# kanster/moped

Measured on AMD Instinct MI355X. Metric: detections/sec (frames/s) 640x480 ~3k SIFT vs N models, higher is better.
Workload: dtype f32

## Files before the change

include/moped_hip.h:

```cpp
#ifndef MOPED_HIP_H
#define MOPED_HIP_H

#include <stddef.h>
#include <stdint.h>

#ifdef __cplusplus
extern "C" {
#endif

#define MH_DESC_DIM 128
#define MH_MAX_BATCH 32
#define MH_MAX_IMAGES 8
#define MH_MAX_MODELS 8192
#define MH_OK 0
#define MH_ERR_ARG (-1)
#define MH_ERR_HIP (-2)
#define MH_ERR_CAPACITY (-3)
#define MH_ERR_NODEVICE (-4)

typedef struct mh_ctx mh_ctx;


int mh_create(int device, mh_ctx** out);
void mh_destroy(mh_ctx* ctx);
// ... 23 lines not shown
int mh_match_stats(mh_ctx* ctx, int Q, uint32_t stats[4], int reset);
int mh_match_set_mode(mh_ctx* ctx, int mode);
int mh_pose_set_split(mh_ctx* ctx, int on);
int mh_match_launches(mh_ctx* ctx, uint32_t out[3]);
float mh_screen_margin(float qq, float dmax);
int mh_screen_values(mh_ctx* ctx, const float* q_host, int Q, int n_rows, float* out_host, float* dmax, float* spread,
                     int shape );
uint16_t mh_screen_record_value(float top, float thr);
void mh_screen_record_bounds(uint16_t value_bits, uint32_t row0, float tau, float spread, int N, float dmax, float* lo,
                             float* hi);
float mh_screen_pack_value(float v, uint32_t id, int bits);
float mh_screen_pack_pert(float qq, float dmax, int bits);
void mh_screen_sample_bounds(uint16_t value_bits, float tau, float pert, float dmax, float* lo, float* hi);
void mh_screen_launch_plan(int Q, int q_expected, int N, int32_t out[8]);
int mh_match_incomplete(mh_ctx* ctx, uint32_t* count, int reset);

int mh_match_local_dev(mh_ctx* ctx, const float* qn_dev, const float* qnorm_dev, int Q,
                       int32_t* idx1_dev, float* d1_dev, float* d2_dev);
int mh_match_merge_dev(mh_ctx* ctx, const int32_t* idx1_s_dev, const float* d1_s_dev,
                       const float* d2_s_dev, int n_shards, int Q,
                       int32_t* idx1_dev, float* d1_dev, float* d2_dev);
int mh_normalize_dev(mh_ctx* ctx, float* q_dev, float* qnorm_dev, int Q);


int mh_meanshift(mh_ctx* ctx, const float* pts_host, int n, int dim, float radius,
                 float merge, int min_pts, int max_iter, int32_t* label,
                 int32_t* order, int32_t* n_clusters);
int mh_meanshift_batch(mh_ctx* ctx, const float* pts_host, const int32_t* off, int n_problems,
                       int dim, float radius, float merge, int min_pts, int max_iter,
                       int32_t* label, int32_t* order, int32_t* n_clusters);
// ... 295 lines not shown
```

moped_amd/capi.py:

```python
from __future__ import annotations

import ctypes as C
import os

import numpy as np

_HERE = os.path.dirname(os.path.abspath(__file__))
LIB_PATH = os.environ.get("MH_LIB_PATH") or os.path.join(_HERE, "libmoped_hip.so")

MH_OK = 0


class MhError(RuntimeError):
    pass


class mh_corr(C.Structure):
    _fields_ = [("u", C.c_float), ("v", C.c_float), ("x", C.c_float), ("y", C.c_float), ("z", C.c_float)]


class mh_cam(C.Structure):
    _fields_ = [("K", C.c_float * 4), ("cam", C.c_float * 7)]


# ... 78 lines not shown
    "mh_db_upload_raw", "mh_db_share", "mh_match_stats", "mh_match_set_mode", "mh_match_launches", "mh_pose_set_split", "mh_frame_fetch_match_points", "mh_screen_margin", "mh_frame_counters", "mh_match_timing", "mh_frame_set_images", "mh_filter_images",
    "mh_pose_ransac_images",
    "mh_comm_unique_id", "mh_comm_create", "mh_comm_create_all", "mh_comm_create_host", "mh_comm_destroy", "mh_comm_info",
    "mh_frame_enqueue_sharded", "mh_frame_enqueue_sharded_batch", "mh_frame_enqueue_sharded_all",
    "mh_frame_previous_objects", "mh_frame_gather_objects", "mh_frame_enqueue_batch", "mh_frame_set_depth_image_batch",
    "mh_pose_kernel_info", "mh_db_upload_blocks", "mh_frame_fetch_matches_slot", "mh_frame_fetch_match_reps_slot",
    "mh_screen_values", "mh_screen_record_value", "mh_screen_record_bounds", "mh_reserve_batch", "mh_frame_run_host",
    "mh_frame_block_stride", "mh_frame_fetch_batch_async", "mh_frame_fetch_previous_async", "mh_frame_fetch_wait",
    "mh_frame_fetch_query", "mh_host_alloc", "mh_host_free", "mh_frame_run_host_begin", "mh_frame_wait_descriptors",
    "mh_step_match", "mh_step_match_fetch", "mh_step_cluster", "mh_step_pose", "mh_step_filter",
    "mh_set_linkage_scratch_limit",
    "mh_undistort_map", "mh_undistort", "mh_undistort_dev", "mh_frame_set_undistort",
    "mh_sift_extract_batch_dev", "mh_sift_debug_plan", "mh_sift_debug_level", "mh_sift_debug_candidates",
    "mh_sift_debug_keys", "mh_sift_debug_blur",
    "mh_screen_pack_value", "mh_screen_pack_pert", "mh_screen_sample_bounds", "mh_screen_launch_plan", "mh_match_incomplete",
]
COMM_ID_BYTES = 128
EX2_OBJECTS = 62
ALLGATHER_FN = C.CFUNCTYPE(C.c_int, C.c_void_p, C.c_void_p, C.c_void_p, C.c_size_t)

_lib = None


def load():
    global _lib
    if _lib is not None:
        return _lib
    try:
        import torch
    except Exception:
# ... 135 lines not shown
    L.mh_screen_values.argtypes = [vp, vp, i32, i32, vp, C.POINTER(f32), C.POINTER(f32), i32]
    L.mh_screen_record_value.argtypes = [f32, f32]
    L.mh_screen_record_value.restype = C.c_uint16
    L.mh_screen_record_bounds.argtypes = [C.c_uint16, C.c_uint32, f32, f32, i32, f32, C.POINTER(f32), C.POINTER(f32)]
    L.mh_screen_record_bounds.restype = None
    if hasattr(L, "mh_screen_pack_value"):
        L.mh_screen_pack_value.argtypes = [f32, C.c_uint32, i32]
        L.mh_screen_pack_value.restype = f32
        L.mh_screen_pack_pert.argtypes = [f32, f32, i32]
        L.mh_screen_pack_pert.restype = f32
        L.mh_screen_sample_bounds.argtypes = [C.c_uint16, f32, f32, f32, C.POINTER(f32), C.POINTER(f32)]
        L.mh_screen_sample_bounds.restype = None
        L.mh_screen_launch_plan.argtypes = [i32, i32, i32, vp]
        L.mh_screen_launch_plan.restype = None
        L.mh_match_incomplete.argtypes = [vp, C.POINTER(C.c_uint32), i32]
    L.mh_db_upload_blocks.argtypes = [vp, vp, vp, vp, i32, i32, vp, vp, i32, i32]
    L.mh_frame_block_stride.argtypes = [i32]
    L.mh_frame_block_stride.restype = C.c_size_t
    L.mh_frame_fetch_batch_async.argtypes = [vp, i32, i32, vp, C.c_uint32]
    L.mh_frame_fetch_previous_async.argtypes = [vp, i32, vp, C.c_uint32]
    L.mh_frame_fetch_wait.argtypes = [vp, C.POINTER(C.c_int32)]
    L.mh_host_alloc.argtypes = [vp, C.c_size_t, C.POINTER(vp)]
    L.mh_host_free.argtypes = [vp, vp]
    L.mh_frame_wait_descriptors.argtypes = [vp]
    if hasattr(L, "mh_step_match"):
        L.mh_set_linkage_scratch_limit.argtypes = [vp, C.c_size_t]
        L.mh_step_match.argtypes = [vp, vp, vp, i32, C.POINTER(mh_cam), f32, i32]
        L.mh_step_match_fetch.argtypes = [vp, vp, vp, vp, i32, C.POINTER(C.c_int32)]
        L.mh_step_cluster.argtypes = [vp, f32, f32, i32, i32, vp, vp, vp, i32, i32, C.POINTER(C.c_int32)]
        L.mh_step_pose.argtypes = [vp, i32, C.POINTER(mh_pose_params), C.c_uint64, vp, i32, C.POINTER(C.c_int32)]
# ... 263 lines not shown
                "waves_per_simd": int(o[3]) * waves / 4.0}

    def match_timing(self) -> dict:
        t = np.zeros(5, np.float32)
        self._ck(self.L.mh_match_timing(self.h, _ptr(t)), "mh_match_timing")
        return dict(zip(("prepare_ms", "pass_a_ms", "thresholds_ms", "pass_b_ms", "pass_c_ms"), (float(v) for v in t)))

    def screen_values(self, qn, n_rows, shape=0):
        qn = np.ascontiguousarray(qn, np.float32)
        out = np.zeros((qn.shape[0], n_rows), np.float32)
        dmax, spread = C.c_float(0), C.c_float(0)
        self._ck(self.L.mh_screen_values(self.h, _ptr(qn), qn.shape[0], n_rows, _ptr(out), C.byref(dmax), C.byref(spread),
                                         int(shape)), "mh_screen_values")
        return out, dmax.value, spread.value

    def match_set_mode(self, mode: int):
        self._ck(self.L.mh_match_set_mode(self.h, int(mode)), "mh_match_set_mode")

    def pose_set_split(self, on: bool):
        self._ck(self.L.mh_pose_set_split(self.h, int(bool(on))), "mh_pose_set_split")

    def match_kernel_launches(self) -> dict:
        o = np.zeros(3, np.uint32)
        self._ck(self.L.mh_match_launches(self.h, _ptr(o)), "mh_match_launches")
        return {"valu": int(o[0]), "mfma": int(o[1]), "screen": int(o[2])}

    def match_stats(self, Q=0, reset=False) -> dict:
        st = np.zeros(4, np.uint32)
        self._ck(self.L.mh_match_stats(self.h, int(Q), _ptr(st), int(reset)), "mh_match_stats")
        return {"candidates": int(st[0]), "brute_force_queries": int(st[1]), "queries": int(st[2]),
                "two_stage": bool(st[3])}

    def match_incomplete(self, reset=False) -> int:
        n = C.c_uint32(0)
        self._ck(self.L.mh_match_incomplete(self.h, C.byref(n), int(reset)), "mh_match_incomplete")
        return int(n.value)

    def normalize(self, desc):
        d = np.ascontiguousarray(desc, np.float32).copy()
        self._ck(self.L.mh_normalize(self.h, _ptr(d), d.shape[0]), "mh_normalize")
        return d

    def match(self, q, ratio=0.8):
        q = np.ascontiguousarray(q, np.float32)
        Q = q.shape[0]
        acc = np.full(Q, -1, np.int32)
# ... 701 lines not shown
```

moped_amd/csrc/api.hip:

```cpp
#include <algorithm>
#include <cmath>
#include <cstring>
#include <new>
#include <vector>

#include "context.h"
#include "steps.h"

using namespace mh;

namespace mh {

int use_stream(mh_ctx* ctx) {
  if (ctx->stream) return MH_OK;
  if (!ctx->own_stream) MH_HIP(ctx, hipStreamCreateWithFlags(&ctx->own_stream, hipStreamNonBlocking));
  ctx->stream = ctx->own_stream;
  return MH_OK;
}

int ensure_scratch(mh_ctx* ctx, size_t bytes) {
  if (bytes <= ctx->scratch_cap) return MH_OK;
  if (ctx->scratch) MH_HIP(ctx, hipFree(ctx->scratch));
  ctx->scratch = nullptr;
  ctx->scratch_cap = 0;
// ... 626 lines not shown
  hipMemcpyAsync(qd, q_host, (size_t)Q * DIM * 4, hipMemcpyHostToDevice, ctx->stream);
  launch_row_norms(qd, qn, Q, ctx->stream);
  launch_screen_prepare(qd, qn, Q, q_pad, qh, qbad, ctx->stream);
  launch_screen_values(qh, Q, ctx->sdb, n_rows, out, ctx->stream, shape);
  if (hipMemcpyAsync(out_host, out, (size_t)Q * n_rows * 4, hipMemcpyDeviceToHost, ctx->stream) != hipSuccess ||
      hipStreamSynchronize(ctx->stream) != hipSuccess || hipGetLastError() != hipSuccess) {
    ctx->err = "mh_screen_values: device error";
    rc = MH_ERR_HIP;
  }
  done();
  if (dmax) *dmax = ctx->sdb.dmax;
  if (spread) *spread = ctx->sdb.spread;
  return rc;
}

int mh_match_set_mode(mh_ctx* ctx, int mode) {
  if (!ctx || mode < -1 || mode > 3) return MH_ERR_ARG;
  ctx->match_mode = mode;
  return MH_OK;
}

int mh_pose_set_split(mh_ctx* ctx, int on) {
  if (!ctx) return MH_ERR_ARG;
  ctx->pose_split = on ? 1 : 0;
  return MH_OK;
}

int mh_match_launches(mh_ctx* ctx, uint32_t out[3]) {
  if (!ctx || !out) return MH_ERR_ARG;
  for (int k = 0; k < 3; ++k) out[k] = ctx->match_launches[k];
// ... 7 lines not shown
  stats[0] = stats[1] = stats[2] = stats[3] = 0;
  if (Q > 0) {
    int rc = ensure_match_scratch(ctx, Q);
    if (rc) return rc;
    stats[3] = (ctx->sdb.usable && ctx->sbuf.q_pad >= screen_q_pad(Q) && screen_wanted(Q, ctx->N, ctx->match_mode >= 2 ? 0 : ctx->match_mode)) ? 1u : 0u;
  }
  MH_HIP(ctx, hipStreamSynchronize(ctx->stream));
  if (ctx->sbuf.stats) {
    std::vector<unsigned int> h((size_t)ctx->sbuf.q_pad * 3);
    MH_HIP(ctx, hipMemcpy(h.data(), ctx->sbuf.stats, h.size() * sizeof(unsigned int), hipMemcpyDeviceToHost));
    unsigned long long sum[3] = {0, 0, 0};
    for (size_t i = 0; i < h.size(); ++i) sum[i % 3] += h[i];
    for (int k = 0; k < 3; ++k) stats[k] = (uint32_t)std::min<unsigned long long>(sum[k], 0xFFFFFFFFull);
    if (reset) MH_HIP(ctx, hipMemset(ctx->sbuf.stats, 0, h.size() * sizeof(unsigned int)));
  }
  return MH_OK;
}

int mh_enable_timing(mh_ctx* ctx, int on) {
  if (!ctx) return MH_ERR_ARG;
  MH_HIP(ctx, hipSetDevice(ctx->device));
  if (int rc_stream = mh::use_stream(ctx)) return rc_stream;
  if (on && !ctx->ev_made) {
    for (auto& e : ctx->ev) MH_HIP(ctx, hipEventCreate(&e));
    for (auto& set : ctx->mev)
      for (auto& e : set) MH_HIP(ctx, hipEventCreate(&e));
    ctx->ev_made = true;
  }
  ctx->timing = on != 0;
  ctx->mev_next = ctx->mev_used = 0;
// ... 24 lines not shown
```

moped_amd/csrc/match_screen.hip:

```cpp
#include <hip/hip_fp16.h>

#include <algorithm>
#include <cstdlib>

#include "common.h"
#include "screen.h"

MH_TRACE_TU()

namespace mh {

namespace {

typedef _Float16 half8 __attribute__((ext_vector_type(8)));
typedef float v16f __attribute__((ext_vector_type(16)));
#define MH_AS1 __attribute__((address_space(1)))
#define MH_AS3 __attribute__((address_space(3)))

constexpr int SC_QPAD = 3 * 1024;
constexpr int SC_TILE = 128;
constexpr int SC_TILE_BYTES = SC_TILE * DIM * 2;
constexpr bool SC_SHAPE16_LARGE = true;
constexpr int SC_NW_LARGE = 8;
__host__ __device__ constexpr int sc_recbuf(int nw) { return nw >= 8 ? 112 : 40; }
// ... 212 lines not shown

constexpr int SC_TOPK = 4;
constexpr int SC_PART5 = SC_TOPK + 1;
constexpr int SC_SA_SPLITS_MAX = 28;
constexpr int SC_PACK_BITS_MAX = 10;
constexpr float SC_PACK_FLOOR = -1e38f;
constexpr unsigned SC_REC_LAYOUT16 = 0x80000000u;
constexpr unsigned SC_REC_SAMPLE = 0x40000000u;

struct SampleGeom {
  int sa_slots;
  int pack_bits;
  int tile_first, tile_stride, tiles_base, tiles_rem, n_sel;
};

__global__ void screen_handover_kernel(const float* __restrict__ part5, int n_lane_slots, int q_pad, int Q,
                                       const int32_t* __restrict__ q_count, const float* __restrict__ qnorm,
                                       const uint8_t* __restrict__ qbad, float dmax, SampleGeom g, float* __restrict__ tau,
                                       uint2* __restrict__ recs, unsigned int* __restrict__ inc) {
  MH_TRACE_SCOPE(mh::TK_TAU);
  const int q = blockIdx.x * blockDim.x + threadIdx.x;
  if (q >= q_pad) return;
  const int Qe = q_count ? min(Q, *q_count) : Q;
  float t = __builtin_inff();
  unsigned incw = 0;
  if (q < Qe && !qbad[q]) {
    auto val = [&](int ls, int k) {
      const float v = part5[((size_t)ls * SC_PART5 + k) * q_pad + q];
      return v < 0.5f * SC_PACK_FLOOR ? -__builtin_inff() : v;
    };
    float B = -__builtin_inff(), S = -__builtin_inff();
#pragma unroll 4
    for (int ls = 0; ls < n_lane_slots; ++ls) {
      const float p1 = val(ls, 0), p2 = val(ls, 1);
      S = fmaxf(fminf(B, p1), fmaxf(S, p2));
      B = fmaxf(B, p1);
    }
    const float P = screen_pack_pert(qnorm[q], dmax, g.pack_bits);
    t = S - P - screen_margin(qnorm[q], dmax);
    if (g.sa_slots > 0 && t > -__builtin_inff()) {
      const float thr = t - P;
      unsigned sm = 0, qm = 0;
#pragma unroll 4
      for (int ls = 0; ls < n_lane_slots; ++ls)
        if (val(ls, SC_TOPK) > thr) {
          sm |= 1u << (ls >> 2);
          qm |= 1u << (ls & 3);
        }
      uint2* mine = recs + (size_t)q * SC_SLOT_PITCH + SC_SLOTS_MAX;
      const unsigned id_mask = (1u << g.pack_bits) - 1u;
      int n = 0;
      bool full = false;
      for (int ls = 0; ls < n_lane_slots && !full; ++ls) {
        const int split = ls >> 2, quarter = ls & 3;
        if (((sm >> split) & 1u) && ((qm >> quarter) & 1u)) continue;
        for (int k = 0; k < SC_TOPK; ++k) {
          const float v = val(ls, k);
          if (!(v > thr)) break;
          if (n == g.sa_slots) {
            full = true;
            break;
          }
          const unsigned id = __float_as_uint(v) & id_mask;
          const int sel = split * g.tiles_base + min(split, g.tiles_rem) + (int)(id >> 2);
          const unsigned row0 = (unsigned)((g.tile_first + sel * g.tile_stride) * SC_TILE + (int)(id & 3u) * 32 + 4 * quarter);
          mine[n++] = make_uint2(row0 | SC_REC_LAYOUT16 | SC_REC_SAMPLE, 0xFFu | ((unsigned)screen_record_value(v, t) << 16));
        }
      }
      if (full) {
        for (int j = 0; j < n; ++j) mine[j] = make_uint2(0u, 0u);
        sm = (1u << (n_lane_slots >> 2)) - 1u;
        qm = 0xFu;
      }
      if (sm) incw = sm | (qm << 28);
    }
  }
  tau[q] = t;
  if (inc) inc[q] = incw;
}

__device__ __forceinline__ void dma16x4(unsigned voff, const void* b0, const void* b1, const void* b2, const void* b3,
                                        unsigned l0, unsigned l1, unsigned l2, unsigned l3) {
  unsigned keep;
  asm volatile(
      "s_mov_b32 %0, m0\n\t"
      "s_mov_b32 m0, %6\n\ts_nop 0\n\tglobal_load_lds_dwordx4 %1, %2\n\t"
      "s_mov_b32 m0, %7\n\ts_nop 0\n\tglobal_load_lds_dwordx4 %1, %3\n\t"
      "s_mov_b32 m0, %8\n\ts_nop 0\n\tglobal_load_lds_dwordx4 %1, %4\n\t"
      "s_mov_b32 m0, %9\n\ts_nop 0\n\tglobal_load_lds_dwordx4 %1, %5\n\t"
      "s_mov_b32 m0, %0"
      : "=&s"(keep)
      : "v"(voff), "s"(b0), "s"(b1), "s"(b2), "s"(b3), "s"(l0), "s"(l1), "s"(l2), "s"(l3)
      : "memory");
// ... 636 lines not shown
    const float4 y2 = *reinterpret_cast<const float4*>(q_lds + 16 * c + 8), y3 = *reinterpret_cast<const float4*>(q_lds + 16 * c + 12);
    s = fmaf(y0.x, x0.x, s); s = fmaf(y0.y, x0.y, s); s = fmaf(y0.z, x0.z, s); s = fmaf(y0.w, x0.w, s);
    s = fmaf(y1.x, x1.x, s); s = fmaf(y1.y, x1.y, s); s = fmaf(y1.z, x1.z, s); s = fmaf(y1.w, x1.w, s);
    s = fmaf(y2.x, x2.x, s); s = fmaf(y2.y, x2.y, s); s = fmaf(y2.z, x2.z, s); s = fmaf(y2.w, x2.w, s);
    s = fmaf(y3.x, x3.x, s); s = fmaf(y3.y, x3.y, s); s = fmaf(y3.z, x3.z, s); s = fmaf(y3.w, x3.w, s);
  }
  return fmaxf(fmaf(-2.f, s, nq + dn), 0.f);
}

__device__ __forceinline__ void wave_lds_sync() {
  __builtin_amdgcn_fence(__ATOMIC_RELEASE, "wavefront");
  __builtin_amdgcn_wave_barrier();
  __builtin_amdgcn_fence(__ATOMIC_ACQUIRE, "wavefront");
}

__global__ __launch_bounds__(64 * RS_WAVES) void rescore_kernel(
    const float* __restrict__ qn, const float* __restrict__ qnorm, const uint8_t* __restrict__ qbad, int Q,
    const int32_t* __restrict__ q_count, const float* __restrict__ db, const float* __restrict__ dnorm, int N,
    RowMap rmap, uint2* __restrict__ recs, int n_slots, int32_t* __restrict__ ovf_cnt, uint2* __restrict__ ovf,
    int ovf_cap, float dmax, const float* __restrict__ tau, float spread, int32_t* __restrict__ idx1, float* __restrict__ d1, float* __restrict__ d2,
    unsigned int* __restrict__ stats, int32_t zero_idx, float zero_d1, float zero_d2, SampleGeom g,
    const unsigned int* __restrict__ inc, unsigned int* __restrict__ inc_count) {
  MH_TRACE_SCOPE(mh::TK_PASS_C);
  __shared__ __attribute__((aligned(16))) float q_s[RS_WAVES][DIM];
  __shared__ __attribute__((aligned(16))) int cand_s[RS_WAVES][RS_MAXC];
  __shared__ int ncand_s[RS_WAVES];
  const int lane = threadIdx.x & 63;
  const int wave = __builtin_amdgcn_readfirstlane(threadIdx.x >> 6);
  const int q = blockIdx.x * RS_WAVES + wave;
  if (q >= Q) return;
  constexpr int RS_ITERS = (SC_SLOT_PITCH + SCREEN_OVF_CAP + 63) / 64;
  uint2* mine = recs + (size_t)q * SC_SLOT_PITCH;
  const int n_own = n_slots + g.sa_slots;
  auto slot_at = [&](int j) -> uint2& { return mine[j < n_slots ? j : SC_SLOTS_MAX + (j - n_slots)]; };
  uint2 recv[RS_ITERS];
#pragma unroll
  for (int it = 0; it < RS_ITERS; ++it) {
    const int j = it * 64 + lane;
    recv[it] = j < n_own ? slot_at(j) : make_uint2(0u, 0u);
  }
  const int Qe = q_count ? min(Q, *q_count) : Q;
// ... 17 lines not shown
      idx1[q] = -1;
      d1[q] = __builtin_inff();
      d2[q] = __builtin_inff();
    }
    return;
  }
  if (bad == 3) {
    if (lane == 0) {
      idx1[q] = zero_idx >= 0 ? row_to_global(rmap, zero_idx) : -1;
      d1[q] = zero_d1;
      d2[q] = zero_d2;
      if (stats) stats[3 * q + 2] += 1u;
    }
    return;
  }
  if (lane == 0) ncand_s[wave] = 0;
  q_s[wave][2 * lane] = qv.x;
  q_s[wave][2 * lane + 1] = qv.y;
  bool brute = n_ovf > ovf_cap || bad == 1;
  int n_cand = 0;
  if (!brute) {
    float l1 = -__builtin_inff(), l2 = -__builtin_inff();
    const float pert = screen_pack_pert(nq, dmax, g.pack_bits);
    auto bounds = [tau_q, spread, N, dmax, pert](uint2 rec, float& lo, float& hi) {
      if (rec.x & SC_REC_SAMPLE) screen_sample_bounds((unsigned short)(rec.y >> 16), tau_q, pert, dmax, lo, hi);
      else screen_record_bounds((unsigned short)(rec.y >> 16), rec.x & 0x3FFFFFFFu, tau_q, spread, N, dmax, lo, hi);
    };
#pragma unroll
    for (int it = 0; it < RS_ITERS; ++it) {
      const int j = it * 64 + lane;
      uint2 rec = recv[it];
// ... 16 lines not shown
      l2 = fmaxf(fmaxf(l2, o2), fminf(l1, o1));
      l1 = fmaxf(l1, o1);
    }
    const float keep_from = l2 - screen_margin(nq, dmax);
#pragma unroll
    for (int it = 0; it < RS_ITERS; ++it) {
      const uint2 rec = recv[it];
      unsigned bits = rec.y & 0xFFFFu;
      if (bits) {
        float lo, hi;
        bounds(rec, lo, hi);
        if (hi < keep_from) bits = 0;
      }
      const int hi_stride = (rec.x & 0x80000000u) ? 16 : 8;
      const int row0 = (int)(rec.x & 0x3FFFFFFFu);
      while (bits) {
        const int r = __builtin_ctz(bits);
        bits &= bits - 1;
        const int w = atomicAdd(&ncand_s[wave], 1);
        if (w < RS_MAXC) cand_s[wave][w] = row0 + (r & 3) + hi_stride * (r >> 2);
      }
    }
    wave_lds_sync();
    n_cand = ncand_s[wave];
    if (n_cand > RS_MAXC) brute = true;
  } else if (n_ovf > ovf_cap) {
    for (int j = lane; j < n_own; j += 64) slot_at(j) = make_uint2(0u, 0u);
  }
  if (n_ovf && lane == 0) ovf_cnt[q] = 0;
  wave_lds_sync();

  Best best = {__builtin_inff(), __builtin_inff(), -1};
  const int n_rows = brute ? N : n_cand;
  if (!brute && n_cand <= 64) {
    const int my_row = lane < n_cand ? cand_s[wave][lane] : -1;
    const bool my_ok = my_row >= 0 && my_row < N;
    const float my_dn = my_ok ? dnorm[my_row] : 0.f;
    wave_lds_sync();
// ... 101 lines not shown
    a[s] = *reinterpret_cast<const half8*>(arow + 16 * s);
    b[s] = *reinterpret_cast<const half8*>(brow + 16 * s);
  }
  v16f acc;
#pragma unroll
  for (int r = 0; r < 16; ++r) {
    const int row = r0 + (r & 3) + 8 * (r >> 2) + 4 * half;
    acc[r] = dneg[(size_t)(row >> 7) * SC_DD + (row & 127)];
  }
#pragma unroll
  for (int s = 0; s < 8; ++s) acc = __builtin_amdgcn_mfma_f32_32x32x16_f16(a[s], b[s], acc, 0, 0, 0);
#pragma unroll
  for (int r = 0; r < 16; ++r) out[(size_t)(q0 + l32) * n_rows + r0 + (r & 3) + 8 * (r >> 2) + 4 * half] = acc[r];
}


}

#ifdef SC_PROF
extern "C" int mh_debug_screen_trace(unsigned long long* out ) {
  return hipMemcpyFromSymbol(out, HIP_SYMBOL(g_sc_trace), 2 * 1024 * sizeof(unsigned long long)) == hipSuccess ? 0 : -1;
}
extern "C" int mh_debug_screen_prof(unsigned long long out[8], int reset, int ablate) {
  if (hipMemcpyFromSymbol(out, HIP_SYMBOL(g_sc_prof), 8 * sizeof(unsigned long long)) != hipSuccess) return -1;
  if (reset) {
    unsigned long long z[8] = {};
    if (hipMemcpyToSymbol(HIP_SYMBOL(g_sc_prof), z, sizeof z) != hipSuccess) return -1;
  }
  g_sc_ablate = ablate;
  return 0;
// ... 8 lines not shown
void launch_db_to_half(const float* db, const float* dnorm, int N, _Float16* dbh, float* dneg, unsigned int* stats,
                       hipStream_t s) {
  const size_t n_chunks = screen_db_half_elems(N) / 8;
  if (n_chunks == 0) return;
  const unsigned blocks = (unsigned)std::min<size_t>((n_chunks + 255) / 256, 2048);
  hipLaunchKernelGGL(db_to_half_kernel, dim3(blocks), dim3(256), 0, s, db, dnorm, N, n_chunks, dbh, dneg, stats);
  const int n_tiles = (int)(n_chunks * 8 / ((size_t)SC_TILE * DIM));
  hipLaunchKernelGGL(db_block_bounds_kernel, dim3((n_tiles * 4 + 255) / 256), dim3(256), 0, s, dnorm, N, n_tiles, dneg, stats);
  hipLaunchKernelGGL(db_zero_query_kernel, dim3(1), dim3(1024), 0, s, dnorm, N, stats);
}

void launch_screen_values(const _Float16* qh, int Q, const ScreenDb& sdb, int n_rows, float* out, hipStream_t s, int shape) {
  if (Q <= 0 || n_rows <= 0) return;
  const int shape16 = shape == 2 || (shape == 0 && SC_SHAPE16_LARGE);
  hipLaunchKernelGGL(screen_values_kernel, dim3(Q / 32, n_rows / 32), dim3(64), 0, s, qh, sdb.dbh, sdb.dneg, n_rows, out, shape16);
}
void launch_screen_prepare(const float* qn, const float* qnorm, int Q, int q_pad, _Float16* qh, uint8_t* qbad, hipStream_t s) {
  hipLaunchKernelGGL(screen_prepare_kernel, dim3((q_pad * 16 + 255) / 256), dim3(256), 0, s, qn, qnorm, Q, (const int32_t*)nullptr,
                     q_pad, qh, qbad);
}

size_t screen_rec_slots() { return SC_SLOT_PITCH; }

int screen_q_pad(int Q) { return (Q + SC_QPAD - 1) / SC_QPAD * SC_QPAD; }
int screen_max_splits_a() { return 64; }
size_t screen_part_bytes(int q_pad) {
  return (size_t)q_pad * std::max<size_t>(screen_max_splits_a() * sizeof(float2), (size_t)SC_SA_SPLITS_MAX * 4 * SC_PART5 * sizeof(float));
}

bool screen_wanted(int q_expected, int N, int mode) {
// ... 117 lines not shown
  attr1.ensure(screen16_kernel<1, NQB>, SC_LDS16_BYTES);
  const int nqb = (Q + QB - 1) / QB;
  const Plan16 p = plan_passes16<NQB>(qe, n_tiles, sample, blocks_a, blocks_b);
  a.n_sel = p.n_sel_a;
  a.tile_first = p.tile_first;
  a.tile_stride = p.stride;
  a.n_splits = p.Sa;
  a.tiles_base = p.n_sel_a / p.Sa;
  a.tiles_rem = p.n_sel_a % p.Sa;
  a.n_splits_a = p.Sa;
  a.pack_keep = ~((1u << p.pack_bits) - 1u);
  a.skip_first = a.skip_stride = 0;
  hipLaunchKernelGGL((screen16_kernel<0, NQB>), dim3(nqb * p.Sa), dim3(512), SC_LDS16_BYTES, s, a);
  if (ev) hipEventRecord(ev[2], s);
  SampleGeom g = {p.onesweep ? SC_SA_SLOTS : 0, p.pack_bits, a.tile_first, a.tile_stride, a.tiles_base, a.tiles_rem, a.n_sel};
  hipLaunchKernelGGL(screen_handover_kernel, dim3((a.q_pad + 63) / 64), dim3(64), 0, s, (const float*)a.part5, 4 * p.Sa, a.q_pad,
                     a.Q, a.q_count, a.qnorm, a.qbad, a.dmax, g, const_cast<float*>(a.tau), a.recs, inc);
#ifdef MH_EXPERIMENTS
  if (exp_int("MH_SCREEN_NO_HITS", 0)) hipMemsetAsync(const_cast<float*>(a.tau), 0x7f, (size_t)a.q_pad * sizeof(float), s);
#endif
  if (ev) hipEventRecord(ev[3], s);
  a.n_sel = p.n_sel_b;
  a.tile_first = 0;
  a.tile_stride = 1;
  a.skip_first = p.onesweep ? p.tile_first : 0;
  a.skip_stride = p.onesweep ? p.stride : 0;
  a.n_splits = p.Sb;
  a.tiles_base = p.n_sel_b / p.Sb;
  a.tiles_rem = p.n_sel_b % p.Sb;
  a.sub_cap = p.sub_cap;
  hipLaunchKernelGGL((screen16_kernel<1, NQB>), dim3(nqb * p.Sb), dim3(512), SC_LDS16_BYTES, s, a);
  if (ev) hipEventRecord(ev[4], s);
// ... 90 lines not shown
  if (shape.passes16 && nqb_sel == 4) launch_passes16<4>(a, Q, qe, n_tiles, sample, blocks_a, blocks_b, &n_slots, &geom, sb.inc, sb.ev, sbig);
  else if (shape.passes16) launch_passes16<2>(a, Q, qe, n_tiles, sample, blocks_a, blocks_b, &n_slots, &geom, sb.inc, sb.ev, sbig);
  else if (nqb_sel == 4 && nw_sel == 4) launch_passes<4, 4>(a, Q, qe, n_tiles, sample, blocks_a, blocks_b, &n_slots, sb.ev, sbig, 256);
  else if (nqb_sel == 4) launch_passes<4, 8>(a, Q, qe, n_tiles, sample, blocks_a, blocks_b, &n_slots, sb.ev, sbig, 256);
  else if (nqb_sel == 3) launch_passes<3, 8>(a, Q, qe, n_tiles, sample, blocks_a, blocks_b, &n_slots, sb.ev, sbig, 256);
  else if (nqb_sel == 2 && nw_sel == 4) launch_passes<2, 4>(a, Q, qe, n_tiles, sample, blocks_a, blocks_b, &n_slots, sb.ev, sbig, 256);
  else if (nqb_sel == 2) launch_passes<2, 8>(a, Q, qe, n_tiles, sample, blocks_a, blocks_b, &n_slots, sb.ev, sbig, 256);
  else launch_passes<1, 8>(a, Q, qe, n_tiles, sample, blocks_a, blocks_b, &n_slots, sb.ev, sbig, 256);
  if (sbig != s) {
    hipEventRecord(sb.ev_out, sbig);
    hipStreamWaitEvent(s, sb.ev_out, 0);
  }
  hipLaunchKernelGGL(rescore_kernel, dim3((Q + RS_WAVES - 1) / RS_WAVES), dim3(64 * RS_WAVES), 0, s, qn, qnorm, sb.qbad, Q,
                     q_count, db, dnorm, N, rmap, sb.recs, n_slots, sb.ovf_cnt, sb.ovf, sb.ovf_cap, sdb.dmax, (const float*)sb.tau, sdb.spread, idx1, d1, d2,
                     sb.stats, sdb.zero_idx, sdb.zero_d1, sdb.zero_d2, geom, geom.sa_slots > 0 ? (const unsigned int*)sb.inc : nullptr,
                     sb.inc ? sb.inc + sb.q_pad : nullptr);
  if (sb.ev) hipEventRecord(sb.ev[5], s);
}

}
```

moped_amd/csrc/screen.h:

```cpp
#pragma once
#include <hip/hip_fp16.h>
#include <hip/hip_runtime.h>
#include <stdint.h>

namespace mh {

struct ScreenDb {
  const _Float16* dbh = nullptr;
  const float* dneg = nullptr;
  float dmax = 0.f;
  float spread = __builtin_inff();
  bool usable = false;
  int32_t zero_idx = -1;
  float zero_d1 = __builtin_inff(), zero_d2 = __builtin_inff();
};

struct ScreenBufs {
  _Float16* qh = nullptr;
  uint8_t* qbad = nullptr;
  float2* part = nullptr;
  float* tau = nullptr;
  uint2* recs = nullptr;
  int32_t* ovf_cnt = nullptr;
  uint2* ovf = nullptr;
// ... 40 lines not shown
                                                     float& hi) {
  _Float16 h;
  __builtin_memcpy(&h, &value_bits, 2);
  const float dv = (float)h;
  const float eps = fabsf(dv) * 0.001f + 1e-6f + 4e-7f * (fabsf(tau_q) + 0.5f * dmax * dmax);
  const bool fin = fabsf(dv) < 6.0e4f && fabsf(tau_q) < 1e30f;
  hi = fin ? tau_q + dv + eps + pert : __builtin_inff();
  lo = fin ? tau_q + dv - eps - pert : -__builtin_inff();
}

constexpr int SCREEN_OVF_CAP = 64;
size_t screen_rec_slots();

float screen_margin_host(float qq, float dmax);
void launch_screen_values(const _Float16* qh, int Q, const ScreenDb& sdb, int n_rows, float* out, hipStream_t s, int shape);
void launch_screen_prepare(const float* qn, const float* qnorm, int Q, int q_pad, _Float16* qh, uint8_t* qbad, hipStream_t s);
size_t screen_db_half_elems(int N);
size_t screen_dneg_elems(int N);
void launch_db_to_half(const float* db, const float* dnorm, int N, _Float16* dbh, float* dneg, unsigned int* stats,
                       hipStream_t s);
int screen_q_pad(int Q);
int screen_max_splits_a();
size_t screen_part_bytes(int q_pad);
void screen_launch_plan(int Q, int q_expected, int N, int out[8]);
bool screen_wanted(int q_expected, int N, int mode = -1);
void launch_match_screen(const float* qn, const float* qnorm, int Q, const float* db, const float* dnorm, int N,
                         const RowMap& rmap, const ScreenDb& sdb, const ScreenBufs& sb, int32_t* idx1, float* d1,
                         float* d2, hipStream_t s, const int32_t* q_count, int q_expected);

}
// ... 1 lines not shown
```

Baseline: 16010.

## Parallelize screen handover across lane-slot parts and prefilter sample records with f16 MFMA

```diff
diff --git a/include/moped_hip.h b/include/moped_hip.h
--- a/include/moped_hip.h
+++ b/include/moped_hip.h
@@ -61,6 +61,8 @@
 void mh_screen_sample_bounds(uint16_t value_bits, float tau, float pert, float dmax, float* lo, float* hi);
 void mh_screen_launch_plan(int Q, int q_expected, int N, int32_t out[8]);
 int mh_match_incomplete(mh_ctx* ctx, uint32_t* count, int reset);
+int mh_screen_sample_values(mh_ctx* ctx, const float* q_host, int Q, const int32_t* row0_host, float* out_host);
+int mh_match_query_candidates(mh_ctx* ctx, int Q, uint32_t* out);
 
 int mh_match_local_dev(mh_ctx* ctx, const float* qn_dev, const float* qnorm_dev, int Q,
                        int32_t* idx1_dev, float* d1_dev, float* d2_dev);
diff --git a/moped_amd/capi.py b/moped_amd/capi.py
--- a/moped_amd/capi.py
+++ b/moped_amd/capi.py
@@ -116,6 +116,7 @@
     "mh_sift_extract_batch_dev", "mh_sift_debug_plan", "mh_sift_debug_level", "mh_sift_debug_candidates",
     "mh_sift_debug_keys", "mh_sift_debug_blur",
     "mh_screen_pack_value", "mh_screen_pack_pert", "mh_screen_sample_bounds", "mh_screen_launch_plan", "mh_match_incomplete",
+    "mh_screen_sample_values", "mh_match_query_candidates",
 ]
 COMM_ID_BYTES = 128
 EX2_OBJECTS = 62
@@ -281,6 +282,9 @@
         L.mh_screen_launch_plan.argtypes = [i32, i32, i32, vp]
         L.mh_screen_launch_plan.restype = None
         L.mh_match_incomplete.argtypes = [vp, C.POINTER(C.c_uint32), i32]
+    if hasattr(L, "mh_screen_sample_values"):
+        L.mh_screen_sample_values.argtypes = [vp, vp, i32, vp, vp]
+        L.mh_match_query_candidates.argtypes = [vp, i32, vp]
     L.mh_db_upload_blocks.argtypes = [vp, vp, vp, vp, i32, i32, vp, vp, i32, i32]
     L.mh_frame_block_stride.argtypes = [i32]
     L.mh_frame_block_stride.restype = C.c_size_t
@@ -574,6 +578,14 @@
                                          int(shape)), "mh_screen_values")
         return out, dmax.value, spread.value
 
+    def screen_sample_values(self, qn, row0):
+        qn = np.ascontiguousarray(qn, np.float32)
+        row0 = np.ascontiguousarray(row0, np.int32)
+        assert row0.shape == (qn.shape[0], 2)
+        out = np.zeros((qn.shape[0], 2, 8), np.float32)
+        self._ck(self.L.mh_screen_sample_values(self.h, _ptr(qn), qn.shape[0], _ptr(row0), _ptr(out)), "mh_screen_sample_values")
+        return out
+
     def match_set_mode(self, mode: int):
         self._ck(self.L.mh_match_set_mode(self.h, int(mode)), "mh_match_set_mode")
 
@@ -590,6 +602,11 @@
         self._ck(self.L.mh_match_stats(self.h, int(Q), _ptr(st), int(reset)), "mh_match_stats")
         return {"candidates": int(st[0]), "brute_force_queries": int(st[1]), "queries": int(st[2]),
                 "two_stage": bool(st[3])}
+
+    def match_query_candidates(self, Q):
+        out = np.zeros(int(Q), np.uint32)
+        self._ck(self.L.mh_match_query_candidates(self.h, int(Q), _ptr(out)), "mh_match_query_candidates")
+        return out
 
     def match_incomplete(self, reset=False) -> int:
         n = C.c_uint32(0)
diff --git a/moped_amd/csrc/api.hip b/moped_amd/csrc/api.hip
--- a/moped_amd/csrc/api.hip
+++ b/moped_amd/csrc/api.hip
@@ -664,6 +664,47 @@
   return rc;
 }
 
+int mh_screen_sample_values(mh_ctx* ctx, const float* q_host, int Q, const int32_t* row0_host, float* out_host) {
+  if (!ctx || !q_host || !row0_host || !out_host || Q <= 0) return MH_ERR_ARG;
+  if (!ctx->sdb.dbh) {
+    ctx->err = "mh_screen_sample_values: the database has no f16 image (fewer than 4096 rows?)";
+    return MH_ERR_ARG;
+  }
+  const int n_pad = (ctx->N + 127) / 128 * 128;
+  for (int i = 0; i < 2 * Q; ++i) {
+    const int r = row0_host[i];
+    if (r < 0 || (r & 3) || (r & 31) >= 16 || r + 19 >= n_pad) {
+      ctx->err = "mh_screen_sample_values: row0 is not the first row of a lane's block (32 b + 4 quarter) inside the padded DB";
+      return MH_ERR_ARG;
+    }
+  }
+  MH_HIP(ctx, hipSetDevice(ctx->device));
+  if (int rc_stream = mh::use_stream(ctx)) return rc_stream;
+  float *qd = nullptr, *out = nullptr;
+  int32_t* rd = nullptr;
+  int rc = MH_OK;
+  auto done = [&]() {
+    for (void* p : {(void*)qd, (void*)out, (void*)rd})
+      if (p) hipFree(p);
+  };
+  if (hipMalloc(&qd, (size_t)Q * DIM * 4) != hipSuccess || hipMalloc(&out, (size_t)Q * 16 * 4) != hipSuccess ||
+      hipMalloc(&rd, (size_t)Q * 2 * 4) != hipSuccess) {
+    done();
+    ctx->err = "mh_screen_sample_values: out of device memory";
+    return MH_ERR_HIP;
+  }
+  hipMemcpyAsync(qd, q_host, (size_t)Q * DIM * 4, hipMemcpyHostToDevice, ctx->stream);
+  hipMemcpyAsync(rd, row0_host, (size_t)Q * 2 * 4, hipMemcpyHostToDevice, ctx->stream);
+  launch_screen_sample_values(qd, Q, ctx->sdb, rd, out, ctx->stream);
+  if (hipMemcpyAsync(out_host, out, (size_t)Q * 16 * 4, hipMemcpyDeviceToHost, ctx->stream) != hipSuccess ||
+      hipStreamSynchronize(ctx->stream) != hipSuccess || hipGetLastError() != hipSuccess) {
+    ctx->err = "mh_screen_sample_values: device error";
+    rc = MH_ERR_HIP;
+  }
+  done();
+  return rc;
+}
+
 int mh_match_set_mode(mh_ctx* ctx, int mode) {
   if (!ctx || mode < -1 || mode > 3) return MH_ERR_ARG;
   ctx->match_mode = mode;
@@ -701,6 +742,21 @@
     for (int k = 0; k < 3; ++k) stats[k] = (uint32_t)std::min<unsigned long long>(sum[k], 0xFFFFFFFFull);
     if (reset) MH_HIP(ctx, hipMemset(ctx->sbuf.stats, 0, h.size() * sizeof(unsigned int)));
   }
+  return MH_OK;
+}
+
+int mh_match_query_candidates(mh_ctx* ctx, int Q, uint32_t* out) {
+  if (!ctx || !out || Q <= 0) return MH_ERR_ARG;
+  MH_HIP(ctx, hipSetDevice(ctx->device));
+  if (int rc_stream = mh::use_stream(ctx)) return rc_stream;
+  MH_HIP(ctx, hipStreamSynchronize(ctx->stream));
+  if (!ctx->sbuf.stats || Q > ctx->sbuf.q_pad) {
+    ctx->err = "mh_match_query_candidates: no two-stage scratch for that many queries";
+    return MH_ERR_ARG;
+  }
+  std::vector<unsigned int> h((size_t)Q * 3);
+  MH_HIP(ctx, hipMemcpy(h.data(), ctx->sbuf.stats, h.size() * sizeof(unsigned int), hipMemcpyDeviceToHost));
+  for (int q = 0; q < Q; ++q) out[q] = h[3 * (size_t)q];
   return MH_OK;
 }
 
diff --git a/moped_amd/csrc/match_screen.hip b/moped_amd/csrc/match_screen.hip
--- a/moped_amd/csrc/match_screen.hip
+++ b/moped_amd/csrc/match_screen.hip
@@ -250,69 +250,117 @@
   int tile_first, tile_stride, tiles_base, tiles_rem, n_sel;
 };
 
-__global__ void screen_handover_kernel(const float* __restrict__ part5, int n_lane_slots, int q_pad, int Q,
-                                       const int32_t* __restrict__ q_count, const float* __restrict__ qnorm,
-                                       const uint8_t* __restrict__ qbad, float dmax, SampleGeom g, float* __restrict__ tau,
-                                       uint2* __restrict__ recs, unsigned int* __restrict__ inc) {
+constexpr int HO_PARTS_MAX = 16;
+template <int HS>
+__global__ __launch_bounds__(64 * HO_PARTS_MAX) void screen_handover_kernel(
+    const float* __restrict__ part5, int n_lane_slots, int q_pad, int Q, const int32_t* __restrict__ q_count,
+    const float* __restrict__ qnorm, const uint8_t* __restrict__ qbad, float dmax, SampleGeom g, float* __restrict__ tau,
+    uint2* __restrict__ recs, unsigned int* __restrict__ inc) {
   MH_TRACE_SCOPE(mh::TK_TAU);
-  const int q = blockIdx.x * blockDim.x + threadIdx.x;
-  if (q >= q_pad) return;
+  __shared__ float s_b[HO_PARTS_MAX][64], s_s[HO_PARTS_MAX][64];
+  __shared__ int s_cnt[HO_PARTS_MAX][64];
+  __shared__ unsigned s_sm[64], s_qm[64];
+  const int ql = threadIdx.x, part = threadIdx.y, n_parts = blockDim.y;
+  const int q = blockIdx.x * 64 + ql;
   const int Qe = q_count ? min(Q, *q_count) : Q;
-  float t = __builtin_inff();
-  unsigned incw = 0;
-  if (q < Qe && !qbad[q]) {
-    auto val = [&](int ls, int k) {
-      const float v = part5[((size_t)ls * SC_PART5 + k) * q_pad + q];
-      return v < 0.5f * SC_PACK_FLOOR ? -__builtin_inff() : v;
-    };
-    float B = -__builtin_inff(), S = -__builtin_inff();
-#pragma unroll 4
-    for (int ls = 0; ls < n_lane_slots; ++ls) {
-      const float p1 = val(ls, 0), p2 = val(ls, 1);
-      S = fmaxf(fminf(B, p1), fmaxf(S, p2));
-      B = fmaxf(B, p1);
-    }
-    const float P = screen_pack_pert(qnorm[q], dmax, g.pack_bits);
-    t = S - P - screen_margin(qnorm[q], dmax);
-    if (g.sa_slots > 0 && t > -__builtin_inff()) {
-      const float thr = t - P;
-      unsigned sm = 0, qm = 0;
-#pragma unroll 4
-      for (int ls = 0; ls < n_lane_slots; ++ls)
-        if (val(ls, SC_TOPK) > thr) {
-          sm |= 1u << (ls >> 2);
-          qm |= 1u << (ls & 3);
-        }
-      uint2* mine = recs + (size_t)q * SC_SLOT_PITCH + SC_SLOTS_MAX;
-      const unsigned id_mask = (1u << g.pack_bits) - 1u;
-      int n = 0;
-      bool full = false;
-      for (int ls = 0; ls < n_lane_slots && !full; ++ls) {
-        const int split = ls >> 2, quarter = ls & 3;
-        if (((sm >> split) & 1u) && ((qm >> quarter) & 1u)) continue;
-        for (int k = 0; k < SC_TOPK; ++k) {
-          const float v = val(ls, k);
-          if (!(v > thr)) break;
-          if (n == g.sa_slots) {
-            full = true;
-            break;
-          }
-          const unsigned id = __float_as_uint(v) & id_mask;
+  const bool live = q < q_pad && q < Qe && !qbad[q];
+  const int ls0 = part * HS;
+  float v[HS][SC_PART5];
+#pragma unroll
+  for (int j = 0; j < HS; ++j)
+#pragma unroll
+    for (int k = 0; k < SC_PART5; ++k)
+      v[j][k] = live && ls0 + j < n_lane_slots ? part5[((size_t)(ls0 + j) * SC_PART5 + k) * q_pad + q] : -__builtin_inff();
+  const float qq = live ? qnorm[q] : 0.f;
+  if (part == 0) {
+    s_sm[ql] = 0u;
+    s_qm[ql] = 0u;
+  }
+  float B = -__builtin_inff(), S = -__builtin_inff();
+#pragma unroll
+  for (int j = 0; j < HS; ++j) {
+#pragma unroll
+    for (int k = 0; k < SC_PART5; ++k) v[j][k] = v[j][k] < 0.5f * SC_PACK_FLOOR ? -__builtin_inff() : v[j][k];
+    S = fmaxf(fminf(B, v[j][0]), fmaxf(S, v[j][1]));
+    B = fmaxf(B, v[j][0]);
+  }
+  s_b[part][ql] = B;
+  s_s[part][ql] = S;
+  __syncthreads();
+  B = S = -__builtin_inff();
+  for (int p = 0; p < n_parts; ++p) {
+    const float ob = s_b[p][ql], os = s_s[p][ql];
+    S = fmaxf(fminf(B, ob), fmaxf(S, os));
+    B = fmaxf(B, ob);
+  }
+  const float P = screen_pack_pert(qq, dmax, g.pack_bits);
+  const float t = live ? S - P - screen_margin(qq, dmax) : __builtin_inff();
+  const float thr = t - P;
+  const bool hand = live && g.sa_slots > 0 && t > -__builtin_inff();
+  unsigned sm = 0, qm = 0;
+  if (hand) {
+#pragma unroll
+    for (int j = 0; j < HS; ++j)
+      if (v[j][SC_TOPK] > thr) {
+        sm |= 1u << ((ls0 + j) >> 2);
+        qm |= 1u << ((ls0 + j) & 3);
+      }
+    if (sm) {
+      atomicOr(&s_sm[ql], sm);
+      atomicOr(&s_qm[ql], qm);
+    }
+  }
+  __syncthreads();
+  sm = s_sm[ql];
+  qm = s_qm[ql];
+  int n_j[HS], cnt = 0;
+#pragma unroll
+  for (int j = 0; j < HS; ++j) {
+    const int ls = ls0 + j;
+    const bool swept = ((sm >> (ls >> 2)) & 1u) && ((qm >> (ls & 3)) & 1u);
+    n_j[j] = 0;
+    bool run = hand && !swept;
+#pragma unroll
+    for (int k = 0; k < SC_TOPK; ++k) {
+      run = run && v[j][k] > thr;
+      n_j[j] += run ? 1 : 0;
+    }
+    cnt += n_j[j];
+  }
+  s_cnt[part][ql] = cnt;
+  __syncthreads();
+  int before = 0, total = 0;
+  for (int p = 0; p < n_parts; ++p) {
+    const int c = s_cnt[p][ql];
+    before += p < part ? c : 0;
+    total += c;
+  }
+  const bool full = total > g.sa_slots;
+  if (cnt && !full) {
+    uint2* mine = recs + (size_t)q * SC_SLOT_PITCH + SC_SLOTS_MAX + before;
+    const unsigned id_mask = (1u << g.pack_bits) - 1u;
+    int n = 0;
+#pragma unroll
+    for (int j = 0; j < HS; ++j) {
+      const int split = (ls0 + j) >> 2, quarter = (ls0 + j) & 3;
+#pragma unroll
+      for (int k = 0; k < SC_TOPK; ++k)
+        if (k < n_j[j]) {
+          const unsigned id = __float_as_uint(v[j][k]) & id_mask;
           const int sel = split * g.tiles_base + min(split, g.tiles_rem) + (int)(id >> 2);
           const unsigned row0 = (unsigned)((g.tile_first + sel * g.tile_stride) * SC_TILE + (int)(id & 3u) * 32 + 4 * quarter);
-          mine[n++] = make_uint2(row0 | SC_REC_LAYOUT16 | SC_REC_SAMPLE, 0xFFu | ((unsigned)screen_record_value(v, t) << 16));
+          mine[n++] = make_uint2(row0 | SC_REC_LAYOUT16 | SC_REC_SAMPLE, 0xFFu | ((unsigned)screen_record_value(v[j][k], t) << 16));
         }
-      }
-      if (full) {
-        for (int j = 0; j < n; ++j) mine[j] = make_uint2(0u, 0u);
-        sm = (1u << (n_lane_slots >> 2)) - 1u;
-        qm = 0xFu;
-      }
-      if (sm) incw = sm | (qm << 28);
-    }
-  }
-  tau[q] = t;
-  if (inc) inc[q] = incw;
+    }
+  }
+  if (part == 0 && q < q_pad) {
+    if (full) {
+      sm = (1u << (n_lane_slots >> 2)) - 1u;
+      qm = 0xFu;
+    }
+    tau[q] = t;
+    if (inc) inc[q] = sm ? sm | (qm << 28) : 0u;
+  }
 }
 
 __device__ __forceinline__ void dma16x4(unsigned voff, const void* b0, const void* b1, const void* b2, const void* b3,
@@ -979,17 +1027,42 @@
   __builtin_amdgcn_fence(__ATOMIC_ACQUIRE, "wavefront");
 }
 
-__global__ __launch_bounds__(64 * RS_WAVES) void rescore_kernel(
+__device__ __forceinline__ v4f sample_pair_values(const float* __restrict__ q_lds, const _Float16* __restrict__ dbh,
+                                                  const float* __restrict__ dneg, int row0x, int row0y, int lane) {
+  const int g = lane >> 4, i = lane & 15;
+  const int arow = (i < 8 ? row0x : row0y) + (i & 3) + 16 * ((i >> 2) & 1);
+  const half8* ap = reinterpret_cast<const half8*>(dbh + (size_t)arow * DIM + 8 * g);
+  half8 a[4];
+#pragma unroll
+  for (int s = 0; s < 4; ++s) a[s] = ap[4 * s];
+  const int crow = (g < 2 ? row0x : row0y) + 16 * (g & 1);
+  const float4 c = *reinterpret_cast<const float4*>(dneg + (size_t)(crow >> 7) * SC_DD + (crow & 127));
+  v4f acc = {c.x, c.y, c.z, c.w};
+#pragma unroll
+  for (int s = 0; s < 4; ++s) {
+    const float4 y0 = *reinterpret_cast<const float4*>(q_lds + 32 * s + 8 * g), y1 = *reinterpret_cast<const float4*>(q_lds + 32 * s + 8 * g + 4);
+    half8 b;
+    b[0] = (_Float16)y0.x; b[1] = (_Float16)y0.y; b[2] = (_Float16)y0.z; b[3] = (_Float16)y0.w;
+    b[4] = (_Float16)y1.x; b[5] = (_Float16)y1.y; b[6] = (_Float16)y1.z; b[7] = (_Float16)y1.w;
+    acc = __builtin_amdgcn_mfma_f32_16x16x32_f16(a[s], b, acc, 0, 0, 0);
+  }
+  return acc;
+}
+
+__global__ __launch_bounds__(64 * RS_WAVES) __attribute__((amdgpu_waves_per_eu(8, 8))) void rescore_kernel(
     const float* __restrict__ qn, const float* __restrict__ qnorm, const uint8_t* __restrict__ qbad, int Q,
     const int32_t* __restrict__ q_count, const float* __restrict__ db, const float* __restrict__ dnorm, int N,
     RowMap rmap, uint2* __restrict__ recs, int n_slots, int32_t* __restrict__ ovf_cnt, uint2* __restrict__ ovf,
     int ovf_cap, float dmax, const float* __restrict__ tau, float spread, int32_t* __restrict__ idx1, float* __restrict__ d1, float* __restrict__ d2,
     unsigned int* __restrict__ stats, int32_t zero_idx, float zero_d1, float zero_d2, SampleGeom g,
-    const unsigned int* __restrict__ inc, unsigned int* __restrict__ inc_count) {
+    const unsigned int* __restrict__ inc, unsigned int* __restrict__ inc_count, const _Float16* __restrict__ dbh,
+    const float* __restrict__ dneg) {
   MH_TRACE_SCOPE(mh::TK_PASS_C);
   __shared__ __attribute__((aligned(16))) float q_s[RS_WAVES][DIM];
   __shared__ __attribute__((aligned(16))) int cand_s[RS_WAVES][RS_MAXC];
   __shared__ int ncand_s[RS_WAVES];
+  __shared__ int samp_s[RS_WAVES][SC_SA_SLOTS];
+  __shared__ int nsamp_s[RS_WAVES];
   const int lane = threadIdx.x & 63;
   const int wave = __builtin_amdgcn_readfirstlane(threadIdx.x >> 6);
   const int q = blockIdx.x * RS_WAVES + wave;
@@ -1037,7 +1110,10 @@
     }
     return;
   }
-  if (lane == 0) ncand_s[wave] = 0;
+  if (lane == 0) {
+    ncand_s[wave] = 0;
+    nsamp_s[wave] = 0;
+  }
   q_s[wave][2 * lane] = qv.x;
   q_s[wave][2 * lane + 1] = qv.y;
   bool brute = n_ovf > ovf_cap || bad == 1;
@@ -1084,6 +1160,11 @@
       }
       const int hi_stride = (rec.x & 0x80000000u) ? 16 : 8;
       const int row0 = (int)(rec.x & 0x3FFFFFFFu);
+      if (bits && (rec.x & SC_REC_SAMPLE)) {
+        const int w = atomicAdd(&nsamp_s[wave], 1);
+        if (w < SC_SA_SLOTS) samp_s[wave][w] = row0;
+        bits = 0;
+      }
       while (bits) {
         const int r = __builtin_ctz(bits);
         bits &= bits - 1;
@@ -1092,6 +1173,24 @@
       }
     }
     wave_lds_sync();
+    const int n_samp = min(nsamp_s[wave], SC_SA_SLOTS), n_pad_rows = (N + SC_TILE - 1) / SC_TILE * SC_TILE;
+    for (int p = 0; p < n_samp; p += 2) {
+      const bool pair = p + 1 < n_samp;
+      const int rx = samp_s[wave][p], ry = samp_s[wave][pair ? p + 1 : p];
+      if (rx + 19 >= n_pad_rows || ry + 19 >= n_pad_rows) continue;
+      const v4f w = sample_pair_values(q_s[wave], dbh, dneg, rx, ry, lane);
+      const int grp = lane >> 4;
+      if ((lane & 15) == 0 && (grp < 2 || pair)) {
+        const int base = (grp < 2 ? rx : ry) + 16 * (grp & 1);
+#pragma unroll
+        for (int r = 0; r < 4; ++r)
+          if (w[r] > tau_q) {
+            const int at = atomicAdd(&ncand_s[wave], 1);
+            if (at < RS_MAXC) cand_s[wave][at] = base + r;
+          }
+      }
+    }
+    if (n_samp) wave_lds_sync();
     n_cand = ncand_s[wave];
     if (n_cand > RS_MAXC) brute = true;
   } else if (n_ovf > ovf_cap) {
@@ -1223,6 +1322,20 @@
   for (int r = 0; r < 16; ++r) out[(size_t)(q0 + l32) * n_rows + r0 + (r & 3) + 8 * (r >> 2) + 4 * half] = acc[r];
 }
 
+__global__ __launch_bounds__(64) void screen_sample_values_kernel(const float* __restrict__ qn, const _Float16* __restrict__ dbh,
+                                                                  const float* __restrict__ dneg, const int32_t* __restrict__ row0,
+                                                                  float* __restrict__ out) {
+  __shared__ __attribute__((aligned(16))) float q_s[DIM];
+  const int lane = threadIdx.x, q = blockIdx.x;
+  const float2 qv = reinterpret_cast<const float2*>(qn + (size_t)q * DIM)[lane];
+  q_s[2 * lane] = qv.x;
+  q_s[2 * lane + 1] = qv.y;
+  __syncthreads();
+  const v4f w = sample_pair_values(q_s, dbh, dneg, row0[2 * q], row0[2 * q + 1], lane);
+  if ((lane & 15) == 0)
+#pragma unroll
+    for (int r = 0; r < 4; ++r) out[(size_t)q * 16 + 4 * (lane >> 4) + r] = w[r];
+}
 
 }
 
@@ -1261,6 +1374,10 @@
   if (Q <= 0 || n_rows <= 0) return;
   const int shape16 = shape == 2 || (shape == 0 && SC_SHAPE16_LARGE);
   hipLaunchKernelGGL(screen_values_kernel, dim3(Q / 32, n_rows / 32), dim3(64), 0, s, qh, sdb.dbh, sdb.dneg, n_rows, out, shape16);
+}
+void launch_screen_sample_values(const float* qn, int Q, const ScreenDb& sdb, const int32_t* row0, float* out, hipStream_t s) {
+  if (Q <= 0) return;
+  hipLaunchKernelGGL(screen_sample_values_kernel, dim3(Q), dim3(64), 0, s, qn, sdb.dbh, sdb.dneg, row0, out);
 }
 void launch_screen_prepare(const float* qn, const float* qnorm, int Q, int q_pad, _Float16* qh, uint8_t* qbad, hipStream_t s) {
   hipLaunchKernelGGL(screen_prepare_kernel, dim3((q_pad * 16 + 255) / 256), dim3(256), 0, s, qn, qnorm, Q, (const int32_t*)nullptr,
@@ -1408,8 +1525,13 @@
   hipLaunchKernelGGL((screen16_kernel<0, NQB>), dim3(nqb * p.Sa), dim3(512), SC_LDS16_BYTES, s, a);
   if (ev) hipEventRecord(ev[2], s);
   SampleGeom g = {p.onesweep ? SC_SA_SLOTS : 0, p.pack_bits, a.tile_first, a.tile_stride, a.tiles_base, a.tiles_rem, a.n_sel};
-  hipLaunchKernelGGL(screen_handover_kernel, dim3((a.q_pad + 63) / 64), dim3(64), 0, s, (const float*)a.part5, 4 * p.Sa, a.q_pad,
-                     a.Q, a.q_count, a.qnorm, a.qbad, a.dmax, g, const_cast<float*>(a.tau), a.recs, inc);
+  static_assert(SC_SA_SPLITS_MAX <= 2 * HO_PARTS_MAX, "a thread of screen_handover_kernel holds at most 8 lane slots");
+  if (p.Sa <= HO_PARTS_MAX)
+    hipLaunchKernelGGL(screen_handover_kernel<4>, dim3((a.q_pad + 63) / 64), dim3(64, p.Sa), 0, s, (const float*)a.part5, 4 * p.Sa,
+                       a.q_pad, a.Q, a.q_count, a.qnorm, a.qbad, a.dmax, g, const_cast<float*>(a.tau), a.recs, inc);
+  else
+    hipLaunchKernelGGL(screen_handover_kernel<8>, dim3((a.q_pad + 63) / 64), dim3(64, (p.Sa + 1) / 2), 0, s, (const float*)a.part5,
+                       4 * p.Sa, a.q_pad, a.Q, a.q_count, a.qnorm, a.qbad, a.dmax, g, const_cast<float*>(a.tau), a.recs, inc);
 #ifdef MH_EXPERIMENTS
   if (exp_int("MH_SCREEN_NO_HITS", 0)) hipMemsetAsync(const_cast<float*>(a.tau), 0x7f, (size_t)a.q_pad * sizeof(float), s);
 #endif
@@ -1530,7 +1652,7 @@
   hipLaunchKernelGGL(rescore_kernel, dim3((Q + RS_WAVES - 1) / RS_WAVES), dim3(64 * RS_WAVES), 0, s, qn, qnorm, sb.qbad, Q,
                      q_count, db, dnorm, N, rmap, sb.recs, n_slots, sb.ovf_cnt, sb.ovf, sb.ovf_cap, sdb.dmax, (const float*)sb.tau, sdb.spread, idx1, d1, d2,
                      sb.stats, sdb.zero_idx, sdb.zero_d1, sdb.zero_d2, geom, geom.sa_slots > 0 ? (const unsigned int*)sb.inc : nullptr,
-                     sb.inc ? sb.inc + sb.q_pad : nullptr);
+                     sb.inc ? sb.inc + sb.q_pad : nullptr, sdb.dbh, sdb.dneg);
   if (sb.ev) hipEventRecord(sb.ev[5], s);
 }
 
diff --git a/moped_amd/csrc/screen.h b/moped_amd/csrc/screen.h
--- a/moped_amd/csrc/screen.h
+++ b/moped_amd/csrc/screen.h
@@ -78,6 +78,7 @@
 
 float screen_margin_host(float qq, float dmax);
 void launch_screen_values(const _Float16* qh, int Q, const ScreenDb& sdb, int n_rows, float* out, hipStream_t s, int shape);
+void launch_screen_sample_values(const float* qn, int Q, const ScreenDb& sdb, const int32_t* row0, float* out, hipStream_t s);
 void launch_screen_prepare(const float* qn, const float* qnorm, int Q, int q_pad, _Float16* qh, uint8_t* qbad, hipStream_t s);
 size_t screen_db_half_elems(int N);
 size_t screen_dneg_elems(int N);
```

After: 16430, median of 6. 1.03x the previous value.
